# matteocarnelos/microflow-rs

Measured on AMD Instinct MI355X. Metric: inferences/sec (int8) for person_detect.tflite, higher is better.
Workload: dtype i8; 1 GPU; person_detect.tflite batch=65536 per GPU, predict_inner int8->int8, inputs resident in HBM; per_gpu_batch=65536, global_batch=65536, parallelism=batch shard x1, no data-path collective

## Files before the change

### microflow_rs_amd/build.py

```python
import os
import shutil
import subprocess
import sys

HERE = os.path.dirname(os.path.abspath(__file__))
CSRC = os.path.join(HERE, "csrc")
LIB = os.path.join(HERE, "libmicroflow_amd.so")
SOURCES = ["capi.cpp", "hostmath.cpp", "epi_fma.cpp", "switches.cpp", "tflite.cpp", "model.cpp", "model_groups.cpp", "wimage.cpp", "ops.hip", "fused.hip", "fused_pairs.hip", "fused_heads.hip", "fused_stages.hip", "chain_partition.hip", "k_generic.hip", "k_depthwise.hip",
           "k_pointwise.hip", "k_fused_mm.hip", "k_stage.hip", "k_dwfc.hip", "k_tail3.hip", "k_gemm.hip", "k_rt.hip", "k_quad.hip", "k_quad_mm.hip", "k_chain.hip", "k_pair_band.hip", "k_pair_band_deep.hip", "k_block_band.hip", "k_pair_wz.hip", "k_fc_rt.hip", "k_pool_fc.hip", "k_conv1_fc.hip", "k_fc_f32.hip",
           "k_conv_gemm.hip", "k_conv_pool.hip", "k_conv_maxpool.hip", "k_add.hip", "k_concat.hip", "k_pad.hip", "k_side_join.hip", "k_dw_gemm.hip", "k_fc_sparse.hip", "k_windows.hip", "windows_spec.cpp"]
HEADERS = ["mf_internal.hpp", "model_groups.hpp", "windows_spec.hpp", "mf_switches.hpp", "ops_impl.hpp", "fused_impl.hpp", "wimage.hpp", "kernels.hpp", "k_common.hpp", "k_add.hpp", "k_concat.hpp", "k_fc_layer.hpp", "k_fc_rt_body.hpp", "k_pool_fc_body.hpp", "k_dwtask.hpp", "k_tail.hpp", "k_pair_band_body.hpp", "k_pair_band_body.inc", "k_conv_rows_body.inc", "k_conv_pool_body.inc", "conv_rows_bytes_map.hpp", os.path.join("..", "..", "include", "microflow_amd.h")]
FLAGS = ["--offload-arch=gfx950", "-O3", "-std=c++17", "-fPIC", "-ffp-contract=off",
         "-fno-fast-math", "-Wall", "-Wno-unused-result", "-mllvm", "-amdgpu-mfma-vgpr-form=1"]
EXTRA = os.environ.get("MF_EXTRA_HIPCC_FLAGS", "").split()
FLAGS += EXTRA
import re
NONSHIPPING = [f for f in EXTRA if re.match(r"-DMF_\w*(KO|DIAG)\w*(=(?!0$)|$)", f)]


UBENCH_SRC = os.path.join(HERE, "..", "scripts", "ubench", "epi_rate.hip")
UBENCH_LIB = os.path.join(HERE, "..", "scripts", "ubench", "libepi_rate.so")


def hipcc():
    exe = shutil.which("hipcc") or "/opt/rocm/bin/hipcc"
    if not os.path.exists(exe):
        raise RuntimeError("hipcc not found: libmicroflow_amd.so cannot be built")
    return exe


def stale():
    if not os.path.exists(LIB):
        return True
    t = os.path.getmtime(LIB)
    deps = [os.path.join(CSRC, f) for f in SOURCES + HEADERS] + [os.path.abspath(__file__)]
    return any(os.path.getmtime(d) > t for d in deps)


def build_ubench(force=False):
    deps = [UBENCH_SRC, os.path.join(CSRC, "k_common.hpp"), os.path.join(CSRC, "kernels.hpp")]
    if (not force and os.path.exists(UBENCH_LIB)
            and os.path.getmtime(UBENCH_LIB) >= max(os.path.getmtime(d) for d in deps)):
        return UBENCH_LIB
    subprocess.check_call([hipcc()] + [f for f in FLAGS if f != "-Wall"] + ["-Wno-unused-value", "-DMF_UBENCH_LIB", "-DITERS=1024", "-shared", "-x", "hip",
                                                    UBENCH_SRC, "-o", UBENCH_LIB])
    return UBENCH_LIB


def build(force=False, verbose=False):
    if NONSHIPPING:
        sys.stderr.write("\n*** microflow_rs_amd/build.py: NON-SHIPPING BUILD -- %s make kernels that are wrong on purpose. "
                         "Rebuild without MF_EXTRA_HIPCC_FLAGS before running tests or benchmarks. ***\n\n" % " ".join(NONSHIPPING))
    build_ubench(force)
    if not force and not stale():
        return LIB
    objdir = os.path.join(HERE, "build")
    os.makedirs(objdir, exist_ok=True)
    cc = hipcc()
    objs = []
    procs = []
    for src in SOURCES:
        obj = os.path.join(objdir, src + ".o")
        objs.append(obj)
        cmd = [cc] + FLAGS + ["-x", "hip", "-c", os.path.join(CSRC, src), "-o", obj]
        if src == "capi.cpp":
            cmd.insert(1, '-DMF_BUILD_EXTRA="%s"' % " ".join(EXTRA).replace('"', ""))
        if verbose:
            print(" ".join(cmd))
        procs.append((src, subprocess.Popen(cmd, stdout=subprocess.PIPE, stderr=subprocess.STDOUT)))
    for src, p in procs:
        out, _ = p.communicate()
        if p.returncode != 0:
            sys.stderr.write(out.decode(errors="replace"))
            raise RuntimeError("hipcc failed on " + src)
        if verbose and out:
            sys.stdout.write(out.decode(errors="replace"))
    cmd = [cc, "--offload-arch=gfx950", "-shared", "-fPIC", "-o", LIB] + objs
    subprocess.check_call(cmd)
    return LIB


if __name__ == "__main__":
    print(build(force="--force" in sys.argv, verbose=True))
```

### microflow_rs_amd/csrc/fused_stages.hip

```cpp
#include <cstring>

#include "fused_impl.hpp"

namespace mf {

FusedImpl *fused_stage_create(FusedImpl *const *pairs, int npairs) {
    const bool off = switches().no_stage;
    if (off || npairs < 2 || !pairs[0] || pairs[0]->kind != FusedImpl::DWPW) return nullptr;
    const OpSpec &d0 = pairs[0]->a->s;
    const char *nm = k::stage_name(d0.H, d0.W, d0.C, npairs);
    if (!nm) return nullptr;
    for (int i = 0; i < npairs; ++i) {
        const FusedImpl *f = pairs[i];
        if (!f || f->kind != FusedImpl::DWPW) return nullptr;
        const OpSpec &d = f->a->s, &q = f->b->s;
        if (d.H != d0.H || d.W != d0.W || d.C != d0.C || d.sh != 1 || q.N != d0.C) return nullptr;
        if (d.u8 != d0.u8 || q.u8 != d0.u8 || !f->dwpw.dw.magic || !f->dwpw.pw.magic || !f->dwpw.dw.wmm) return nullptr;
        if (f->dwpw.dw.izp4 != pairs[0]->dwpw.dw.izp4 || f->a->device != pairs[0]->a->device) return nullptr;
    }
    bool all_fma = true;
    for (int i = 0; i < npairs; ++i) all_fma = all_fma && pairs[i]->a->fma_ok && pairs[i]->b->fma_ok;
    std::vector<k::EpiPatchRec> ptab((size_t)npairs * 32, k::EpiPatchRec{0, 0});
    for (int i = 0; i < npairs && all_fma; ++i)
        for (int ph = 0; ph < 2 && all_fma; ++ph) {
            const k::EpiPatch &pl = (ph ? pairs[i]->b : pairs[i]->a)->fma_patch;
            for (int e = 0; e < pl.n && all_fma; ++e) {
                const int ch = pl.ch[e];
                if (ch < 0 || ch >= 128) {
                    all_fma = false;
                    break;
                }
                k::EpiPatchRec *slot = &ptab[(((size_t)i * 2 + ph) * 8 + (size_t)(ch >> 4)) * 2];
                if (slot[0].P != 0) ++slot;
                if (slot->P != 0) all_fma = false;
                else *slot = k::epi_patch_rec(pl.P[e], pl.R[e], ch & 3, (ch >> 2) & 3);
                if (all_fma && slot != &ptab[(((size_t)i * 2 + ph) * 8 + (size_t)(ch >> 4)) * 2]) slot[-1].meta |= 32;
            }
        }
    std::unique_ptr<FusedImpl> s = make_group(FusedImpl::STAGE, pairs[0]->a, pairs[npairs - 1]->b, nullptr, nm);
    s->stage.pairs = npairs;
    std::vector<k::StagePair> table((size_t)npairs);
    for (int i = 0; i < npairs; ++i) {
        const OpImpl *dw = pairs[i]->a, *pw = pairs[i]->b;
        const k::DwPwArgs pa = pair_args(dw, pw, all_fma ? 2 : 0);
        k::StagePair &sp = table[(size_t)i];
        set_pair_consts(sp, pa.dw, pa.pw);
        sp.dw_wmm = pa.dw.wmm, sp.dwK = kc_with_magic(*s, host_kc(dw, pa.dw.Kc));
        sp.pw_w = plain_pw_image(*s, pw);
        sp.pwK = kc_with_magic(*s, host_kc(pw, pa.pw.Kc));
    }
    k::StageArgs &a = s->stage.args;
    a.patch_tab = nullptr;
    if (all_fma) {
        a.patch_tab = (const k::EpiPatchRec *)keep(*s, ptab.data(), ptab.size() * sizeof(k::EpiPatchRec));
    }
    a.pairs = (const k::StagePair *)keep(*s, table.data(), table.size() * sizeof(k::StagePair));
    a.izp4 = pairs[0]->dwpw.dw.izp4;
    a.xr4 = d0.u8 ? 0x80808080u : 0u;
    a.queue = pairs[0]->dwpw.dw.queue, a.qlaunch = pairs[0]->dwpw.dw.qlaunch;
    a.mode = all_fma ? 3 : 2;
    for (int i = 0; i < npairs && !all_fma; ++i)
        if (pairs[i]->a->magic_mode != 2 || pairs[i]->b->magic_mode != 2) a.mode = 1;
    s->epi_mode = a.mode;
    return s.release();
}

template <typename T> static void pair_tail_operands(FusedImpl &f, T &a, const OpImpl *dw, const OpImpl *pw, const k::DwFastArgs &df, int magic) {
    set_pair_consts(a, df, pw->conv);
    a.dw_wmm = df.wmm, a.izp4 = df.izp4;
    if (magic) a.dwK = kc_with_magic(f, dw->h_Kc);
    a.pw_w = plain_pw_image(f, pw);
    if (magic) a.pwK = kc_with_magic(f, pw->h_Kc);
}

FusedImpl *fused_pair_tail_create(FusedImpl *pair, FusedImpl *tail) {
    const bool off = switches().no_pairtail;
    if (off || !pair || !tail || tail->kind != FusedImpl::TAIL) return nullptr;
    OpImpl *dw = nullptr, *pw = nullptr;
    if (pair->kind == FusedImpl::DWPW) dw = pair->a, pw = pair->b;
    else if (fused_is_chain_single(pair)) dw = pair->chain.members[0].first, pw = pair->chain.members[0].second;
    const PairMatch m = match_dw3x3_pw1x1(dw, pw);
    if (!m || !m.f || !m.f->wmm || (dw->fast == OpImpl::DW_RT && dw->rt_wz)) return nullptr;
    if ((pw->fast != OpImpl::PW_MFMA && pw->fast != OpImpl::PW_RT) || (pw->fast == OpImpl::PW_RT && pw->rt_wz)) return nullptr;
    const OpSpec &d = *m.d, &q = *m.q;
    const k::TailArgs &t = tail->tail;
    if (!k::pair_tail_supported(d.H, d.W, d.C, q.N, t.N, t.ntaps) || d.sh != 1) return nullptr;
    if ((d.u8 ? 0x80 : 0) != t.xr) return nullptr;
    if (t.H != d.OH || t.W != d.OW || t.C != q.N || dw->device != tail->a->device) return nullptr;
    const int magic = (dw->magic_mode >= 1 && pw->magic_mode >= 1) ? 1 : 0;
    std::unique_ptr<FusedImpl> f = make_group(FusedImpl::PAIRTAIL, dw, tail->b, tail->c, k::pair_tail_name(d.H, d.C));
    k::PairTailArgs &a = f->pairtail.args;
    a.H = d.H, a.C = d.C, a.magic = magic;
    f->epi_mode = magic;
    pair_tail_operands(*f, a, dw, pw, *m.f, magic);
    a.tail = t;
    return f.release();
}

FusedImpl *fused_front_pair_tail_create(FusedImpl *front, FusedImpl *pairtail) {
    if (switches().no_pair_front || !front || !pairtail || pairtail->kind != FusedImpl::PAIRTAIL || pairtail->pairtail.has_front) return nullptr;
    if (front->kind != FusedImpl::DWPW) return nullptr;
    OpImpl *dw = front->a, *pw = front->b;
    const PairMatch m = match_dw3x3_pw1x1(dw, pw);
    if (!m || dw->fast != OpImpl::DW_NHWC || pw->fast != OpImpl::PW_MFMA) return nullptr;
    const OpSpec &d = *m.d, &q = *m.q;
    const k::PairTailArgs &t = pairtail->pairtail.args;
    if (!k::pair_front_supported(d.H, d.W, d.C, d.sh, q.N, t.H, t.C)) return nullptr;
    if (q.OH != t.H || q.OW != t.H || (d.u8 ? 0x80u : 0u) != (uint32_t)t.tail.xr || dw->device != pairtail->a->device) return nullptr;
    if (!m.f->wmm) return nullptr;
    const int magic = (dw->magic_mode >= 1 && pw->magic_mode >= 1) ? 1 : 0;
    if (magic != t.magic) return nullptr;
    std::unique_ptr<FusedImpl> f = make_group(FusedImpl::PAIRTAIL, dw, pairtail->b, pairtail->c, "pair_front_tail<6,6,128,2,256|3,3,256,2>");
    f->pairtail.args = t, f->pairtail.has_front = true, f->epi_mode = magic;
    pair_tail_operands(*f, f->pairtail.front, dw, pw, *m.f, magic);
    return f.release();
}

static std::unique_ptr<FusedImpl> quad_group(FusedImpl *p1, FusedImpl *p2, const k::DwPwArgs &a, const k::DwPwArgs &b, const char *name, bool mm) {
    const OpSpec &d1 = p1->a->s, &q1 = p1->b->s, &d2 = p2->a->s, &q2 = p2->b->s;
    std::unique_ptr<FusedImpl> f = make_group(FusedImpl::QUAD, p1->a, p2->b, nullptr, name);
    f->quad.args.a = a, f->quad.args.b = b, f->quad.mm = mm;
    f->epi_mode = std::min(pair_mode(a), pair_mode(b));
    f->quad.ops[0] = p1->a, f->quad.ops[1] = p1->b, f->quad.ops[2] = p2->a, f->quad.ops[3] = p2->b;
    const int shp[10] = {d1.H, d1.W, d1.C, d1.sh, q1.N, d2.H, d2.W, d2.C, d2.sh, q2.N};
    for (int i = 0; i < 10; ++i) f->quad.shape[i] = shp[i];
    return f;
}
FusedImpl *fused_quad_create(FusedImpl *p1, FusedImpl *p2) {
    const bool off = switches().no_quad;
    if (off || !p1 || !p2 || p1->kind != FusedImpl::DWPW || p2->kind != FusedImpl::DWPW) return nullptr;
    const OpSpec &d1 = p1->a->s, &q1 = p1->b->s, &d2 = p2->a->s, &q2 = p2->b->s;
    if (p1->a->device != p2->a->device || d1.u8 != d2.u8) return nullptr;
    if (d2.H != q1.H || d2.W != q1.W || d2.C != q1.N) return nullptr;
    if (k::quad_mm_shape(d1.H, d1.W, d1.C, d1.sh, q1.N, d2.H, d2.W, d2.C, d2.sh, q2.N)) {
        if (switches().no_quad_mm) return nullptr;
        k::DwPwArgs a = p1->dwpw, b = p2->dwpw;
        if (pair_mode(a) != 3 || pair_mode(b) != 3) a = pair_args(p1->a, p1->b, 0), b = pair_args(p2->a, p2->b, 0);
        if (!a.dw.wmm || !a.pw.wprep || !b.dw.wmm || !b.pw.wprep) return nullptr;
        if (!a.dw.magic || !a.pw.magic || !b.dw.magic || !b.pw.magic) return nullptr;
        return quad_group(p1, p2, a, b, "quad_mm<12,12,64,1,64|12,12,64,2,128>", true).release();
    }
    const char *nm = k::quad_name(d1.H, d1.W, d1.C, d1.sh, q1.N, d2.H, d2.W, d2.C, d2.sh, q2.N);
    if (!nm) return nullptr;
    const bool fma = p1->a->fma_strict() && p1->b->fma_strict() && p2->a->fma_strict() && p2->b->fma_strict();
    const k::DwPwArgs a = pair_args(p1->a, p1->b, fma ? 1 : 0), b = pair_args(p2->a, p2->b, fma ? 1 : 0);
    if (!a.dw.wmm || !a.pw.wrr || !b.dw.wmm || !b.pw.wrr) return nullptr;
    if (!a.dw.magic || !a.pw.magic || !b.dw.magic || !b.pw.magic) return nullptr;
    return quad_group(p1, p2, a, b, nm, false).release();
}

FusedImpl *fused_quad_stem_create(OpImpl *stem, FusedImpl *quad) {
    const bool off = switches().no_penta;
    if (off || !stem || !quad || quad->kind != FusedImpl::QUAD || quad->quad.args.stem || stem->fast != OpImpl::DW_STEM) return nullptr;
    const OpSpec &t = stem->s, &d1 = quad->a->s;
    if (stem->device != quad->a->device || t.u8 != d1.u8 || stem->force_generic) return nullptr;
    if (t.OH != d1.H || t.OW != d1.W || t.N != d1.C || t.sh != 2 || t.sw != 2 || t.C != 1) return nullptr;
    const int *q = quad->quad.shape;
    const char *nm = k::quad_stem_name(t.H, t.W, q[0], q[1], q[2], q[3], q[4], q[5], q[6], q[7], q[8], q[9]);
    if (!nm || !stem->stem.magic) return nullptr;
    std::unique_ptr<FusedImpl> f = make_group(FusedImpl::QUAD, stem, quad->b, nullptr, nm);
    k::QuadArgs &a = f->quad.args;
    a = quad->quad.args;
    for (int i = 0; i < 10; ++i) f->quad.shape[i] = q[i];
    OpImpl *const *qo = quad->quad.ops;
    const bool fma = stem->fma_strict() && qo[0]->fma_strict() && qo[1]->fma_strict() && qo[2]->fma_strict() && qo[3]->fma_strict();
    a.a = pair_args(qo[0], qo[1], fma ? 1 : 0), a.b = pair_args(qo[2], qo[3], fma ? 1 : 0);
    k::DwStemArgs sa = stem->stem;
    if (fma) sa.use_fma();
    std::vector<uint32_t> tab(152);
    for (int l = 0; l < 64; ++l) tab[(size_t)2 * l] = sa.wmm[l][0], tab[(size_t)2 * l + 1] = sa.wmm[l][1];
    for (int c = 0; c < 8; ++c) {
        memcpy(&tab[(size_t)128 + c], &sa.A[c], 4);
        memcpy(&tab[(size_t)136 + c], &sa.S[c], 4);
        memcpy(&tab[(size_t)144 + c], &sa.Kc[c], 4);
    }
    a.stem = (const uint32_t *)keep(*f, tab.data(), tab.size() * 4);
    a.stem_izp4 = sa.izp4, a.stem_lo = sa.lo_f, a.stem_hi = sa.hi_f, a.stem_magic = sa.magic;
    a.in_scale = sa.in_scale, a.in_zp_f = sa.in_zp_f, a.in_sat_lo = sa.in_sat_lo, a.in_sat_hi = sa.in_sat_hi;
    a.in_rcp = sa.in_rcp, a.in_xr4 = sa.in_xr4, a.in_fast = sa.in_fast, a.f32_ok = stem->accepts_f32 ? 1 : 0;
    f->epi_mode = std::min(std::min(pair_mode(a.a), pair_mode(a.b)), sa.magic);
    return f.release();
}

}
```

### microflow_rs_amd/csrc/k_quad_mm.hip

```cpp
#include "k_common.hpp"

#ifndef MF_QMM_UB
#define MF_QMM_UB 2
#endif
#ifndef MF_QMM_KO
#define MF_QMM_KO 0
#endif
namespace mf {
namespace k {

namespace {
struct Q64 {
    static constexpr int G = 2, NTHR = 512, NWAVE = 8, NQ = 4, LP = 64, ROWB = 768;
    static constexpr int ROW_A = LP + ROWB + LP + 16, TILE_A = 14 * ROW_A, BUF_A = G * TILE_A;
    static constexpr int OPIX_A = 144, NPIX_A = G * OPIX_A, PLANE_A = NPIX_A * 16 + 16;
    static constexpr int ROW_B = LP + ROWB + LP, TILE_B = 14 * ROW_B, BUF_B = G * TILE_B, TS_B = 0x043;
    static constexpr int OPIX_B = 36, NPIX_B = G * OPIX_B, P16_B = 80, PLANE_B = P16_B * 16 + 16;
    static constexpr int OFF_TA = 0;
    static constexpr int OFF_MA = OFF_TA + BUF_A + 512;
    static constexpr int OFF_TB = OFF_MA + NQ * PLANE_A + 64;
    static constexpr int OFF_MB = OFF_TB + BUF_B + 512;
    static constexpr int OFF_C = OFF_MB + NQ * PLANE_B + 64;
    static constexpr int C_A_DW = 0, C_A_PW = 64 * 12, C_B_DW = 2 * 64 * 12, C_B_PW = 3 * 64 * 12, C_BYTES = 3 * 64 * 12 + 128 * 12;
    static constexpr int OFF_Q = OFF_C + C_BYTES;
    static constexpr int LDS = OFF_Q + 16;
};
static_assert(2 * Q64::LDS <= 160 * 1024, "two workgroups per CU");
static_assert(Q64::OFF_MA % 16 == 0 && Q64::OFF_TB % 16 == 0 && Q64::OFF_MB % 16 == 0, "16-byte aligned regions");
}

template <int MG, uint32_t XR4>
__global__ __launch_bounds__(512, 4) void quad_mm_12x12x64(const int8_t *__restrict__ in, int8_t *__restrict__ out, QuadArgs p, int batch) {
    using Z = Q64;
    constexpr int UB = MF_QMM_UB;
    epi_enter<MG>();
    extern __shared__ __attribute__((aligned(16))) uint8_t lds[];
    const int tid = threadIdx.x, lane = tid & 63;
    const int wave = __builtin_amdgcn_readfirstlane(tid >> 6);
    DynSteps dq;
    dq.init(lds + Z::OFF_Q, p.a.dw.queue, tid, p.a.dw.qcfg);

    for (int i = tid; i < (Z::BUF_A + 512) / 16; i += Z::NTHR)
        ((uint4 *)(lds + Z::OFF_TA))[i] = make_uint4(p.a.dw.izp4, p.a.dw.izp4, p.a.dw.izp4, p.a.dw.izp4);
    for (int i = tid; i < (Z::BUF_B + 512) / 16; i += Z::NTHR)
        ((uint4 *)(lds + Z::OFF_TB))[i] = make_uint4(p.b.dw.izp4, p.b.dw.izp4, p.b.dw.izp4, p.b.dw.izp4);

    const int col = lane & 15, g = lane >> 4;
    const int qa = wave & 3, ha = wave >> 2;
    const int cyA = col & 3, cxA = col >> 2;
    const int tbA = Z::OFF_TA + ha * Z::TILE_A + cyA * Z::ROW_A + Z::LP + (cxA + g - 1) * 64 + 16 * qa;
    const int mbA = Z::OFF_MA + qa * Z::PLANE_A + (ha * Z::OPIX_A + cyA * 12 + cxA) * 16 + 4 * g;
    const int cxB = col & 7, cyB = col >> 3;
    const int xlB = cxB * 2 + g - 1;
    const int tbB = Z::OFF_TB + ha * Z::TILE_B + cyB * 2 * Z::ROW_B + Z::LP + xlB * 64 + 16 * (qa ^ tile_swz<Z::TS_B>(xlB));
    const int mbB = Z::OFF_MB + qa * Z::PLANE_B + (ha * Z::OPIX_B + cyB * 6 + cxB) * 16 + 4 * g;
    const bool liveB = cxB < 6;
    v4i AdA[3], AdB[3];
#pragma unroll
    for (int ty = 0; ty < 3; ++ty) {
        AdA[ty] = ((const v4i *)p.a.dw.wmm)[(qa * 3 + ty) * 64 + lane];
        AdB[ty] = ((const v4i *)p.b.dw.wmm)[(qa * 3 + ty) * 64 + lane];
    }
    const v4i AwA = ((const v4i *)p.a.pw.wprep)[qa * 64 + lane];
    const int blk = wave >> 2, tt = wave & 3;
    const v4i AwB = ((const v4i *)p.b.pw.wprep)[wave * 64 + lane];
    {
        auto put = [&](int off, int n, const float *A, const float *S, const int *K) {
            for (int i = tid; i < n; i += Z::NTHR) {
                ((float *)(lds + Z::OFF_C + off))[i] = A[i], ((float *)(lds + Z::OFF_C + off))[n + i] = S[i];
                ((int *)(lds + Z::OFF_C + off))[2 * n + i] = K[i] + (MG != 0 ? MF_MAGIC_I : 0);
            }
        };
        put(Z::C_A_DW, 64, p.a.dw.A, p.a.dw.S, p.a.dw.Kc), put(Z::C_A_PW, 64, p.a.pw.A, p.a.pw.S, p.a.pw.Kc);
        put(Z::C_B_DW, 64, p.b.dw.A, p.b.dw.S, p.b.dw.Kc), put(Z::C_B_PW, 128, p.b.pw.A, p.b.pw.S, p.b.pw.Kc);
    }
    struct Consts {
        float4 a, s;
        int4 k;
    };
    auto consts = [&](int off, int n, int ch) {
        Consts c;
        c.a = *(const float4 *)(lds + Z::OFF_C + off + ch * 4), c.s = *(const float4 *)(lds + Z::OFF_C + off + (n + ch) * 4);
        c.k = *(const int4 *)(lds + Z::OFF_C + off + (2 * n + ch) * 4);
        return c;
    };
    const int ch_dw = 16 * qa + 4 * g, chA = g * 16 + 4 * qa, chB = blk * 64 + g * 16 + 4 * tt;
    int oB[9];
#pragma unroll
    for (int c = 0; c < 9; ++c) {
        const int pix = c * 16 + col, y = pix / 12, x = pix - y * 12;
        oB[c] = Z::OFF_TB + ha * Z::TILE_B + (y + 1) * Z::ROW_B + Z::LP + x * 64 + 16 * (g ^ tile_swz<Z::TS_B>(x)) + 4 * qa;
    }
    const EpiPatchRec prDA = epi_patch_load(MG == 3 ? p.a.dw.patch : nullptr, qa), prPA = epi_patch_load(MG == 3 ? p.a.pw.patch : nullptr, qa);
    const EpiPatchRec prDB = epi_patch_load(MG == 3 ? p.b.dw.patch : nullptr, qa), prPB = epi_patch_load(MG == 3 ? p.b.pw.patch : nullptr, wave);
    wg_sync();

    auto stage = [&](int st) {
#pragma unroll
        for (int k = 0; k < 3; ++k) {
            const int r = k * Z::NWAVE + wave, gi = r / 12, y = r % 12;
            if (st * Z::G + gi < batch && lane < 48)
                dma16(in + ((size_t)(st * Z::G + gi) * 9216 + y * Z::ROWB + lane * 16), lds + Z::OFF_TA + gi * Z::TILE_A + (y + 1) * Z::ROW_A + Z::LP);
        }
    };
    auto out_addr = [](int pix, int slot) { return Z::OFF_TB + (pix / 6 + 1) * Z::ROW_B + Z::LP + (pix % 6) * 128 + 16 * (slot ^ (pix & 7)); };
    auto copy_out = [&](int st, int gv) {
        int8_t *ob = out + (size_t)st * Z::G * Z::OPIX_B * 128;
        for (int j = tid; j < gv * Z::OPIX_B * 8; j += Z::NTHR) {
            const int pix = j >> 3, sp = j & 7;
            st_out(ob + pix * 128 + ((sp ^ (pix & 7)) << 4), *(const uint4 *)(lds + Z::OFF_TB + (pix / 6 + 1) * Z::ROW_B + Z::LP + (pix % 6) * 128 + sp * 16));
        }
    };

    const int nsteps = (batch + Z::G - 1) / Z::G;
    if (dq.step < nsteps) stage(dq.step);
    int prev = -1, prev_gv = 0;
    for (; dq.step < nsteps; dq.advance(tid)) {
        const int step = dq.step;
        asm volatile("s_waitcnt vmcnt(0)" ::: "memory");
        wg_sync();
        dq.top(tid);
        const int next = dq.nxt;
        const int gvalid = min(Z::G, batch - step * Z::G);
        if (prev >= 0 && !(MF_QMM_KO & 2)) copy_out(prev, prev_gv);

        {
            constexpr int NU = 9;
            const Consts k = consts(Z::C_A_DW, 64, ch_dw);
            auto toff = [](int t) constexpr { return (t / 3) * 4 * Z::ROW_A + (t % 3) * 4 * 64; };
            v4i bq[UB][3], bn[UB][3];
#pragma unroll
            for (int u = 0; u < UB; ++u)
#pragma unroll
                for (int ty = 0; ty < 3; ++ty) bq[u][ty] = *(const v4i *)(lds + tbA + toff(u < NU ? u : 0) + ty * Z::ROW_A);
#pragma unroll
            for (int t0 = 0; t0 < NU; t0 += UB) {
                v4i acc[UB];
#pragma unroll
                for (int u = 0; u < UB; ++u) acc[u] = v4i{k.k.x, k.k.y, k.k.z, k.k.w};
#pragma unroll
                for (int ty = 0; ty < 3; ++ty)
#pragma unroll
                    for (int u = 0; u < UB; ++u)
                        if (t0 + u < NU) acc[u] = __builtin_amdgcn_mfma_i32_16x16x64_i8(AdA[ty], bq[u][ty], acc[u], 0, 0, 0);
#pragma unroll
                for (int u = 0; u < UB; ++u)
                    if (t0 + UB + u < NU) {
#pragma unroll
                        for (int ty = 0; ty < 3; ++ty) bn[u][ty] = *(const v4i *)(lds + tbA + toff(t0 + UB + u) + ty * Z::ROW_A);
                    }
#pragma unroll
                for (int u = 0; u < UB; ++u)
                    if (t0 + u < NU) {
                        const int t = t0 + u;
                        if constexpr (MG == 3) epi_patch_apply(acc[u], prDA, g);
                        const uint32_t d = (MF_QMM_KO & 16) ? (uint32_t)(acc[u][0] ^ acc[u][1] ^ acc[u][2] ^ acc[u][3])
                                                            : requant_pack4<MG, XR4>(acc[u][0], acc[u][1], acc[u][2], acc[u][3], k.a, k.s, p.a.dw.lo_f, p.a.dw.hi_f);
                        *(uint32_t *)(lds + mbA + ((t / 3) * 4 * 12 + (t % 3) * 4) * 16) = d;
                    }
#pragma unroll
                for (int u = 0; u < UB; ++u)
#pragma unroll
                    for (int ty = 0; ty < 3; ++ty) bq[u][ty] = bn[u][ty];
            }
        }
        wg_sync();
        if (next < nsteps && !((MF_QMM_KO & 8) && prev >= 0)) stage((MF_QMM_KO & 32) ? (int)(blockIdx.x & 63) : next);

        {
            constexpr int NC = 9;
            const Consts k = consts(Z::C_A_PW, 64, chA);
            const uint8_t *mid = lds + Z::OFF_MA + g * Z::PLANE_A + (ha * Z::OPIX_A + col) * 16;
            v4i bq[UB], bn[UB];
#pragma unroll
            for (int u = 0; u < UB; ++u) bq[u] = *(const v4i *)(mid + (u < NC ? u : 0) * 256);
#pragma unroll
            for (int c0 = 0; c0 < NC; c0 += UB) {
                v4i acc[UB];
#pragma unroll
                for (int u = 0; u < UB; ++u)
                    if (c0 + u < NC) acc[u] = __builtin_amdgcn_mfma_i32_16x16x64_i8(AwA, bq[u], v4i{k.k.x, k.k.y, k.k.z, k.k.w}, 0, 0, 0);
#pragma unroll
                for (int u = 0; u < UB; ++u)
                    if (c0 + UB + u < NC) bn[u] = *(const v4i *)(mid + (c0 + UB + u) * 256);
#pragma unroll
                for (int u = 0; u < UB; ++u)
                    if (c0 + u < NC) {
                        if constexpr (MG == 3) epi_patch_apply(acc[u], prPA, g);
                        const uint32_t d = (MF_QMM_KO & 16) ? (uint32_t)(acc[u][0] ^ acc[u][1] ^ acc[u][2] ^ acc[u][3])
                                                            : requant_pack4<MG, XR4>(acc[u][0], acc[u][1], acc[u][2], acc[u][3], k.a, k.s, p.a.pw.lo_f, p.a.pw.hi_f);
                        *(uint32_t *)(lds + oB[c0 + u]) = d;
                    }
#pragma unroll
                for (int u = 0; u < UB; ++u) bq[u] = bn[u];
            }
        }
        if (!(MF_QMM_KO & 1)) wg_sync();

        if (!(MF_QMM_KO & 4)) {
            constexpr int NU = 3;
            const Consts k = consts(Z::C_B_DW, 64, ch_dw);
            v4i bq[NU][3];
#pragma unroll
            for (int t = 0; t < NU; ++t)
#pragma unroll
                for (int ty = 0; ty < 3; ++ty) bq[t][ty] = *(const v4i *)(lds + tbB + (t * 4 + ty) * Z::ROW_B);
            v4i acc[NU];
#pragma unroll
            for (int t = 0; t < NU; ++t) acc[t] = v4i{k.k.x, k.k.y, k.k.z, k.k.w};
#pragma unroll
            for (int ty = 0; ty < 3; ++ty)
#pragma unroll
                for (int t = 0; t < NU; ++t) acc[t] = __builtin_amdgcn_mfma_i32_16x16x64_i8(AdB[ty], bq[t][ty], acc[t], 0, 0, 0);
#pragma unroll
            for (int t = 0; t < NU; ++t) {
                if constexpr (MG == 3) epi_patch_apply(acc[t], prDB, g);
                const uint32_t d = (MF_QMM_KO & 16) ? (uint32_t)(acc[t][0] ^ acc[t][1] ^ acc[t][2] ^ acc[t][3])
                                                    : requant_pack4<MG, XR4>(acc[t][0], acc[t][1], acc[t][2], acc[t][3], k.a, k.s, p.b.dw.lo_f, p.b.dw.hi_f);
                if (liveB) *(uint32_t *)(lds + mbB + t * 2 * 6 * 16) = d;
            }
        }
        if (!(MF_QMM_KO & 1)) wg_sync();

        if (!(MF_QMM_KO & 4)) {
            constexpr int NC = 5;
            const Consts k = consts(Z::C_B_PW, 128, chB);
            v4i b[NC], acc[NC];
#pragma unroll
            for (int c = 0; c < NC; ++c) {
                const int pix = c * 16 + col, pc = pix < Z::NPIX_B ? pix : Z::NPIX_B - 1;
                b[c] = *(const v4i *)(lds + Z::OFF_MB + g * Z::PLANE_B + pc * 16);
            }
#pragma unroll
            for (int c = 0; c < NC; ++c) acc[c] = __builtin_amdgcn_mfma_i32_16x16x64_i8(AwB, b[c], v4i{k.k.x, k.k.y, k.k.z, k.k.w}, 0, 0, 0);
#pragma unroll
            for (int c = 0; c < NC; ++c) {
                const int pix = c * 16 + col;
                if constexpr (MG == 3) epi_patch_apply(acc[c], prPB, g);
                const uint32_t d = (MF_QMM_KO & 16) ? (uint32_t)(acc[c][0] ^ acc[c][1] ^ acc[c][2] ^ acc[c][3])
                                                    : requant_pack4<MG, XR4>(acc[c][0], acc[c][1], acc[c][2], acc[c][3], k.a, k.s, p.b.pw.lo_f, p.b.pw.hi_f);
                if (pix < Z::NPIX_B) *(uint32_t *)(lds + out_addr(pix, blk * 4 + g) + 4 * tt) = d;
            }
        }
        prev = step, prev_gv = gvalid;
    }
    wg_sync();
    if (prev >= 0) copy_out(prev, prev_gv);
    dq.finish(tid);
}

template <int MG, uint32_t XR4> static void launch_quad_mm_t(const int8_t *in, int8_t *out, const QuadArgs &a, int batch, hipStream_t s) {
    static LaunchState st;
    const int per_cu = prepared(st, quad_mm_12x12x64<MG, XR4>, Q64::NTHR, Q64::LDS);
    const int nsteps = (batch + Q64::G - 1) / Q64::G;
    const int grid = nsteps < 256 * per_cu ? nsteps : 256 * per_cu;
    QuadArgs b = a;
    b.a.dw.qcfg = dq_config(nsteps, grid, dq_est_us((double)batch * (9216 + 4608), (double)batch * (9216 * 2 + 2304 + 4608)));
    b.a.dw.queue = dq_slot(b.a.dw.queue, b.a.dw.qlaunch);
    MF_LAUNCH((quad_mm_12x12x64<MG, XR4>), dim3(grid), dim3(Q64::NTHR), Q64::LDS, s, in, out, b, batch);
}
bool quad_mm_shape(int H, int W, int C, int S, int N, int H2, int W2, int C2, int S2, int N2) {
    return H == 12 && W == 12 && C == 64 && S == 1 && N == 64 && H2 == 12 && W2 == 12 && C2 == 64 && S2 == 2 && N2 == 128;
}
void launch_quad_mm(const int8_t *in, int8_t *out, const QuadArgs &a, int batch, hipStream_t s) {
    const int mg = std::min(std::min(a.a.dw.magic, a.a.pw.magic), std::min(a.b.dw.magic, a.b.pw.magic));
    const bool u8 = a.a.dw.xr != 0;
    if (mg == 3) launch_quad_mm_t<3, 0u>(in, out, a, batch, s);
    else if (u8) {
        if (mg == 2) launch_quad_mm_t<2, 0x80808080u>(in, out, a, batch, s);
        else launch_quad_mm_t<1, 0x80808080u>(in, out, a, batch, s);
    } else {
        if (mg == 2) launch_quad_mm_t<2, 0u>(in, out, a, batch, s);
        else launch_quad_mm_t<1, 0u>(in, out, a, batch, s);
    }
}

}
}
```

Measured before the change: 30.60 million inferences/s.

## Make quad_mm pointwise channel tiling contiguous and repad LDS tile-B layout

Moves the quad_mm LDS layout into a shared header and adds a layout mode, on by default, where each wave owns a contiguous 16-channel group for the pointwise stages. It pads tile-B rows by 64 bytes, changes the swizzle bits, and drops the per-plane padding. The apparent goal is fewer LDS bank conflicts on the write and copy-out paths and removal of the clamp on dead-lane mid reads. Because the channel-to-wave mapping changes, the host remaps weight prep indices and epilogue patch tables to match, which adds risk of a mismatch.

Measured after the change: 30.82 million inferences/s (median of 6 runs). No clear change (+0.7%).

```diff
diff --git a/microflow_rs_amd/build.py b/microflow_rs_amd/build.py
--- a/microflow_rs_amd/build.py
+++ b/microflow_rs_amd/build.py
@@ -9,7 +9,7 @@
 SOURCES = ["capi.cpp", "hostmath.cpp", "epi_fma.cpp", "switches.cpp", "tflite.cpp", "model.cpp", "model_groups.cpp", "wimage.cpp", "ops.hip", "fused.hip", "fused_pairs.hip", "fused_heads.hip", "fused_stages.hip", "chain_partition.hip", "k_generic.hip", "k_depthwise.hip",
            "k_pointwise.hip", "k_fused_mm.hip", "k_stage.hip", "k_dwfc.hip", "k_tail3.hip", "k_gemm.hip", "k_rt.hip", "k_quad.hip", "k_quad_mm.hip", "k_chain.hip", "k_pair_band.hip", "k_pair_band_deep.hip", "k_block_band.hip", "k_pair_wz.hip", "k_fc_rt.hip", "k_pool_fc.hip", "k_conv1_fc.hip", "k_fc_f32.hip",
            "k_conv_gemm.hip", "k_conv_pool.hip", "k_conv_maxpool.hip", "k_add.hip", "k_concat.hip", "k_pad.hip", "k_side_join.hip", "k_dw_gemm.hip", "k_fc_sparse.hip", "k_windows.hip", "windows_spec.cpp"]
-HEADERS = ["mf_internal.hpp", "model_groups.hpp", "windows_spec.hpp", "mf_switches.hpp", "ops_impl.hpp", "fused_impl.hpp", "wimage.hpp", "kernels.hpp", "k_common.hpp", "k_add.hpp", "k_concat.hpp", "k_fc_layer.hpp", "k_fc_rt_body.hpp", "k_pool_fc_body.hpp", "k_dwtask.hpp", "k_tail.hpp", "k_pair_band_body.hpp", "k_pair_band_body.inc", "k_conv_rows_body.inc", "k_conv_pool_body.inc", "conv_rows_bytes_map.hpp", os.path.join("..", "..", "include", "microflow_amd.h")]
+HEADERS = ["mf_internal.hpp", "model_groups.hpp", "windows_spec.hpp", "mf_switches.hpp", "ops_impl.hpp", "fused_impl.hpp", "wimage.hpp", "kernels.hpp", "k_common.hpp", "k_quad_mm_layout.hpp", "k_add.hpp", "k_concat.hpp", "k_fc_layer.hpp", "k_fc_rt_body.hpp", "k_pool_fc_body.hpp", "k_dwtask.hpp", "k_tail.hpp", "k_pair_band_body.hpp", "k_pair_band_body.inc", "k_conv_rows_body.inc", "k_conv_pool_body.inc", "conv_rows_bytes_map.hpp", os.path.join("..", "..", "include", "microflow_amd.h")]
 FLAGS = ["--offload-arch=gfx950", "-O3", "-std=c++17", "-fPIC", "-ffp-contract=off",
          "-fno-fast-math", "-Wall", "-Wno-unused-result", "-mllvm", "-amdgpu-mfma-vgpr-form=1"]
 EXTRA = os.environ.get("MF_EXTRA_HIPCC_FLAGS", "").split()
diff --git a/microflow_rs_amd/csrc/fused_stages.hip b/microflow_rs_amd/csrc/fused_stages.hip
--- a/microflow_rs_amd/csrc/fused_stages.hip
+++ b/microflow_rs_amd/csrc/fused_stages.hip
@@ -1,6 +1,7 @@
 #include <cstring>
 
 #include "fused_impl.hpp"
+#include "k_quad_mm_layout.hpp"
 
 namespace mf {
 
@@ -136,9 +137,19 @@
         if (switches().no_quad_mm) return nullptr;
         k::DwPwArgs a = p1->dwpw, b = p2->dwpw;
         if (pair_mode(a) != 3 || pair_mode(b) != 3) a = pair_args(p1->a, p1->b, 0), b = pair_args(p2->a, p2->b, 0);
+        k::EpiPatchRec tab[4 + 8] = {};
+        const bool pa = pair_mode(a) == 3 && a.pw.patch, pb = pair_mode(b) == 3 && b.pw.patch;
+        if ((pa && !k::quad_mm_pw_patch(p1->b->fma_patch, 4, tab)) || (pb && !k::quad_mm_pw_patch(p2->b->fma_patch, 8, tab + 4)))
+            a = pair_args(p1->a, p1->b, 0), b = pair_args(p2->a, p2->b, 0);
         if (!a.dw.wmm || !a.pw.wprep || !b.dw.wmm || !b.pw.wprep) return nullptr;
         if (!a.dw.magic || !a.pw.magic || !b.dw.magic || !b.pw.magic) return nullptr;
-        return quad_group(p1, p2, a, b, "quad_mm<12,12,64,1,64|12,12,64,2,128>", true).release();
+        std::unique_ptr<FusedImpl> f = quad_group(p1, p2, a, b, "quad_mm<12,12,64,1,64|12,12,64,2,128>", true);
+        if (pair_mode(a) == 3 && (pa || pb)) {
+            const k::EpiPatchRec *t = (const k::EpiPatchRec *)keep(*f, tab, sizeof(tab));
+            if (pa) f->quad.args.a.pw.patch = t;
+            if (pb) f->quad.args.b.pw.patch = t + 4;
+        }
+        return f.release();
     }
     const char *nm = k::quad_name(d1.H, d1.W, d1.C, d1.sh, q1.N, d2.H, d2.W, d2.C, d2.sh, q2.N);
     if (!nm) return nullptr;
diff --git a/microflow_rs_amd/csrc/k_quad_mm.hip b/microflow_rs_amd/csrc/k_quad_mm.hip
--- a/microflow_rs_amd/csrc/k_quad_mm.hip
+++ b/microflow_rs_amd/csrc/k_quad_mm.hip
@@ -1,4 +1,5 @@
 #include "k_common.hpp"
+#include "k_quad_mm_layout.hpp"
 
 #ifndef MF_QMM_UB
 #define MF_QMM_UB 2
@@ -8,26 +9,6 @@
 #endif
 namespace mf {
 namespace k {
-
-namespace {
-struct Q64 {
-    static constexpr int G = 2, NTHR = 512, NWAVE = 8, NQ = 4, LP = 64, ROWB = 768;
-    static constexpr int ROW_A = LP + ROWB + LP + 16, TILE_A = 14 * ROW_A, BUF_A = G * TILE_A;
-    static constexpr int OPIX_A = 144, NPIX_A = G * OPIX_A, PLANE_A = NPIX_A * 16 + 16;
-    static constexpr int ROW_B = LP + ROWB + LP, TILE_B = 14 * ROW_B, BUF_B = G * TILE_B, TS_B = 0x043;
-    static constexpr int OPIX_B = 36, NPIX_B = G * OPIX_B, P16_B = 80, PLANE_B = P16_B * 16 + 16;
-    static constexpr int OFF_TA = 0;
-    static constexpr int OFF_MA = OFF_TA + BUF_A + 512;
-    static constexpr int OFF_TB = OFF_MA + NQ * PLANE_A + 64;
-    static constexpr int OFF_MB = OFF_TB + BUF_B + 512;
-    static constexpr int OFF_C = OFF_MB + NQ * PLANE_B + 64;
-    static constexpr int C_A_DW = 0, C_A_PW = 64 * 12, C_B_DW = 2 * 64 * 12, C_B_PW = 3 * 64 * 12, C_BYTES = 3 * 64 * 12 + 128 * 12;
-    static constexpr int OFF_Q = OFF_C + C_BYTES;
-    static constexpr int LDS = OFF_Q + 16;
-};
-static_assert(2 * Q64::LDS <= 160 * 1024, "two workgroups per CU");
-static_assert(Q64::OFF_MA % 16 == 0 && Q64::OFF_TB % 16 == 0 && Q64::OFF_MB % 16 == 0, "16-byte aligned regions");
-}
 
 template <int MG, uint32_t XR4>
 __global__ __launch_bounds__(512, 4) void quad_mm_12x12x64(const int8_t *__restrict__ in, int8_t *__restrict__ out, QuadArgs p, int batch) {
@@ -52,7 +33,7 @@
     const int mbA = Z::OFF_MA + qa * Z::PLANE_A + (ha * Z::OPIX_A + cyA * 12 + cxA) * 16 + 4 * g;
     const int cxB = col & 7, cyB = col >> 3;
     const int xlB = cxB * 2 + g - 1;
-    const int tbB = Z::OFF_TB + ha * Z::TILE_B + cyB * 2 * Z::ROW_B + Z::LP + xlB * 64 + 16 * (qa ^ tile_swz<Z::TS_B>(xlB));
+    const int tbB = q64_tile_b(ha, cyB * 2 - 1, xlB, 16 * qa);
     const int mbB = Z::OFF_MB + qa * Z::PLANE_B + (ha * Z::OPIX_B + cyB * 6 + cxB) * 16 + 4 * g;
     const bool liveB = cxB < 6;
     v4i AdA[3], AdB[3];
@@ -61,9 +42,8 @@
         AdA[ty] = ((const v4i *)p.a.dw.wmm)[(qa * 3 + ty) * 64 + lane];
         AdB[ty] = ((const v4i *)p.b.dw.wmm)[(qa * 3 + ty) * 64 + lane];
     }
-    const v4i AwA = ((const v4i *)p.a.pw.wprep)[qa * 64 + lane];
-    const int blk = wave >> 2, tt = wave & 3;
-    const v4i AwB = ((const v4i *)p.b.pw.wprep)[wave * 64 + lane];
+    const v4i AwA = ((const v4i *)p.a.pw.wprep)[q64_pw_wprep(qa, lane)];
+    const v4i AwB = ((const v4i *)p.b.pw.wprep)[q64_pw_wprep(wave, lane)];
     {
         auto put = [&](int off, int n, const float *A, const float *S, const int *K) {
             for (int i = tid; i < n; i += Z::NTHR) {
@@ -84,12 +64,12 @@
         c.k = *(const int4 *)(lds + Z::OFF_C + off + (2 * n + ch) * 4);
         return c;
     };
-    const int ch_dw = 16 * qa + 4 * g, chA = g * 16 + 4 * qa, chB = blk * 64 + g * 16 + 4 * tt;
+    const int ch_dw = 16 * qa + 4 * g, chA = q64_pw_ch(qa, g), chB = q64_pw_ch(wave, g);
     int oB[9];
 #pragma unroll
     for (int c = 0; c < 9; ++c) {
         const int pix = c * 16 + col, y = pix / 12, x = pix - y * 12;
-        oB[c] = Z::OFF_TB + ha * Z::TILE_B + (y + 1) * Z::ROW_B + Z::LP + x * 64 + 16 * (g ^ tile_swz<Z::TS_B>(x)) + 4 * qa;
+        oB[c] = q64_tile_b(ha, y, x, chA);
     }
     const EpiPatchRec prDA = epi_patch_load(MG == 3 ? p.a.dw.patch : nullptr, qa), prPA = epi_patch_load(MG == 3 ? p.a.pw.patch : nullptr, qa);
     const EpiPatchRec prDB = epi_patch_load(MG == 3 ? p.b.dw.patch : nullptr, qa), prPB = epi_patch_load(MG == 3 ? p.b.pw.patch : nullptr, wave);
@@ -103,12 +83,11 @@
                 dma16(in + ((size_t)(st * Z::G + gi) * 9216 + y * Z::ROWB + lane * 16), lds + Z::OFF_TA + gi * Z::TILE_A + (y + 1) * Z::ROW_A + Z::LP);
         }
     };
-    auto out_addr = [](int pix, int slot) { return Z::OFF_TB + (pix / 6 + 1) * Z::ROW_B + Z::LP + (pix % 6) * 128 + 16 * (slot ^ (pix & 7)); };
     auto copy_out = [&](int st, int gv) {
         int8_t *ob = out + (size_t)st * Z::G * Z::OPIX_B * 128;
         for (int j = tid; j < gv * Z::OPIX_B * 8; j += Z::NTHR) {
             const int pix = j >> 3, sp = j & 7;
-            st_out(ob + pix * 128 + ((sp ^ (pix & 7)) << 4), *(const uint4 *)(lds + Z::OFF_TB + (pix / 6 + 1) * Z::ROW_B + Z::LP + (pix % 6) * 128 + sp * 16));
+            st_out(ob + pix * 128 + ((sp ^ q64_out_xor(pix)) << 4), *(const uint4 *)(lds + q64_out_slot(pix, sp)));
         }
     };
 
@@ -227,10 +206,7 @@
             const Consts k = consts(Z::C_B_PW, 128, chB);
             v4i b[NC], acc[NC];
 #pragma unroll
-            for (int c = 0; c < NC; ++c) {
-                const int pix = c * 16 + col, pc = pix < Z::NPIX_B ? pix : Z::NPIX_B - 1;
-                b[c] = *(const v4i *)(lds + Z::OFF_MB + g * Z::PLANE_B + pc * 16);
-            }
+            for (int c = 0; c < NC; ++c) b[c] = *(const v4i *)(lds + Z::OFF_MB + g * Z::PLANE_B + q64_mid_b_pix(c * 16 + col) * 16);
 #pragma unroll
             for (int c = 0; c < NC; ++c) acc[c] = __builtin_amdgcn_mfma_i32_16x16x64_i8(AwB, b[c], v4i{k.k.x, k.k.y, k.k.z, k.k.w}, 0, 0, 0);
 #pragma unroll
@@ -239,7 +215,7 @@
                 if constexpr (MG == 3) epi_patch_apply(acc[c], prPB, g);
                 const uint32_t d = (MF_QMM_KO & 16) ? (uint32_t)(acc[c][0] ^ acc[c][1] ^ acc[c][2] ^ acc[c][3])
                                                     : requant_pack4<MG, XR4>(acc[c][0], acc[c][1], acc[c][2], acc[c][3], k.a, k.s, p.b.pw.lo_f, p.b.pw.hi_f);
-                if (pix < Z::NPIX_B) *(uint32_t *)(lds + out_addr(pix, blk * 4 + g) + 4 * tt) = d;
+                if (pix < Z::NPIX_B) *(uint32_t *)(lds + q64_out(pix, chB)) = d;
             }
         }
         prev = step, prev_gv = gvalid;
diff --git a/microflow_rs_amd/csrc/k_quad_mm_layout.hpp b/microflow_rs_amd/csrc/k_quad_mm_layout.hpp
--- /dev/null
+++ b/microflow_rs_amd/csrc/k_quad_mm_layout.hpp
@@ -0,0 +1,68 @@
+#pragma once
+#include "kernels.hpp"
+
+#if defined(__HIPCC__)
+#define MF_QMM_HD __host__ __device__ inline constexpr
+#else
+#define MF_QMM_HD inline constexpr
+#endif
+#ifndef MF_QMM_LAYOUT
+#define MF_QMM_LAYOUT 2
+#endif
+
+namespace mf {
+namespace k {
+
+struct Q64 {
+    static constexpr int G = 2, NTHR = 512, NWAVE = 8, NQ = 4, LP = 64, ROWB = 768;
+    static constexpr bool CONTIG = MF_QMM_LAYOUT >= 2;
+    static constexpr int PLANE_PAD = MF_QMM_LAYOUT >= 1 ? 0 : 16;
+    static constexpr int ROW_A = LP + ROWB + LP + 16, TILE_A = 14 * ROW_A, BUF_A = G * TILE_A;
+    static constexpr int OPIX_A = 144, NPIX_A = G * OPIX_A, PLANE_A = NPIX_A * 16 + PLANE_PAD;
+    static constexpr int PAD_B = CONTIG ? 64 : 0, TS_B = CONTIG ? 0x023 : 0x043;
+    static constexpr int ROW_B = LP + ROWB + LP + PAD_B, TILE_B = 14 * ROW_B, BUF_B = G * TILE_B;
+    static constexpr int OPIX_B = 36, NPIX_B = G * OPIX_B, P16_B = 80, PLANE_B = P16_B * 16 + PLANE_PAD;
+    static constexpr int OFF_TA = 0;
+    static constexpr int OFF_MA = OFF_TA + BUF_A + 512;
+    static constexpr int OFF_TB = OFF_MA + NQ * PLANE_A + 64;
+    static constexpr int OFF_MB = OFF_TB + BUF_B + 512;
+    static constexpr int OFF_C = OFF_MB + NQ * PLANE_B + 64;
+    static constexpr int C_A_DW = 0, C_A_PW = 64 * 12, C_B_DW = 2 * 64 * 12, C_B_PW = 3 * 64 * 12, C_BYTES = 3 * 64 * 12 + 128 * 12;
+    static constexpr int OFF_Q = OFF_C + C_BYTES;
+    static constexpr int LDS = OFF_Q + 16;
+};
+static_assert(2 * Q64::LDS <= 160 * 1024, "two workgroups per CU");
+static_assert(Q64::OFF_MA % 16 == 0 && Q64::OFF_TB % 16 == 0 && Q64::OFF_MB % 16 == 0, "16-byte aligned regions");
+static_assert((Q64::TS_B & 0xf) != 0 && (Q64::TS_B >> 4 & 0xf) != 0 && (Q64::TS_B >> 8) == 0, "two swizzle bits: a pixel has four groups");
+
+MF_QMM_HD int q64_swz(int x) { return ((x >> ((Q64::TS_B & 0xf) - 1)) & 1) | ((x >> ((Q64::TS_B >> 4 & 0xf) - 1)) & 1) << 1; }
+
+MF_QMM_HD int q64_pw_ch(int tile, int g) { return Q64::CONTIG ? 16 * tile + 4 * g : (tile >> 2) * 64 + 16 * g + 4 * (tile & 3); }
+MF_QMM_HD int q64_pw_wprep(int tile, int lane) {
+    return Q64::CONTIG ? ((tile & ~3) + ((lane & 15) >> 2)) * 64 + (lane & 48) + 4 * (tile & 3) + (lane & 3) : tile * 64 + lane;
+}
+
+MF_QMM_HD int q64_tile_b(int h, int y, int x, int ch) {
+    return Q64::OFF_TB + h * Q64::TILE_B + (y + 1) * Q64::ROW_B + Q64::LP + x * 64 + 16 * ((ch >> 4) ^ q64_swz(x)) + (ch & 15);
+}
+MF_QMM_HD int q64_out_xor(int pix) { return Q64::CONTIG ? (pix & 7) ^ ((pix / 6 & 1) << 2) : pix & 7; }
+MF_QMM_HD int q64_out_slot(int pix, int phys) { return Q64::OFF_TB + (pix / 6 + 1) * Q64::ROW_B + Q64::LP + (pix % 6) * 128 + 16 * phys; }
+MF_QMM_HD int q64_out(int pix, int ch) { return q64_out_slot(pix, (ch >> 4) ^ q64_out_xor(pix)) + (ch & 15); }
+MF_QMM_HD int q64_mid_b_pix(int pix) { return Q64::CONTIG || pix < Q64::NPIX_B ? pix : Q64::NPIX_B - 1; }
+static_assert(Q64::P16_B * 16 <= Q64::PLANE_B, "the dead lanes' slots lie inside the plane");
+
+inline bool quad_mm_pw_patch(const EpiPatch &pl, int ntiles, EpiPatchRec *tab) {
+    for (int e = 0; e < pl.n; ++e) {
+        const int ch = pl.ch[e];
+        int tile = -1, grp = 0;
+        for (int t = 0; t < ntiles && tile < 0; ++t)
+            for (int g = 0; g < 4; ++g)
+                if ((ch & ~3) == q64_pw_ch(t, g)) tile = t, grp = g;
+        if (tile < 0 || tab[tile].P != 0) return false;
+        tab[tile] = epi_patch_rec(pl.P[e], pl.R[e], ch & 3, grp);
+    }
+    return true;
+}
+
+}
+}
```
